# JohannesBuchner/massivedatans

Hardware: AMD Instinct MI355X
Metric: likelihood evals/sec across N datasets per constrained draw (higher is better)
Workload: dtype f64

## Files before the change

### massivedatans_amd/csrc/mdns_internal.h

```cpp
#pragma once
#include <hip/hip_runtime.h>
#include <cstddef>
#include <cstdint>
#include <cstring>
#include <utility>
#include "mdns.h"

namespace mdns {

void set_error(const char *fmt, ...);
bool hip_ok(hipError_t e, const char *what, const char *file, int line);
#define MDNS_HIP(call) ::mdns::hip_ok((call), #call, __FILE__, __LINE__)
bool launched(const char *name);

enum class Wait { ok, timeout, failed, empty };
Wait wait_seq(const volatile unsigned long long *at, unsigned long long want, hipError_t *err = nullptr);
bool wait_ok(Wait w, hipError_t err, const char *who);

constexpr size_t grown_bytes(size_t need, size_t elem) { return ((need + need / 2) * elem + 4095) / 4096 * 4096; }
static_assert(grown_bytes(0, 8) == 0, "nothing asked, nothing made");
static_assert(grown_bytes(1, 8) == 4096, "one element: one page");
static_assert(grown_bytes(341, 8) == 4096, "341 + 170 doubles = 4088 bytes: still one page");
static_assert(grown_bytes(342, 8) == 8192, "342 + 171 doubles = 4104 bytes: two pages");
constexpr size_t exact_bytes(size_t need, size_t elem) { return (need ? need : 1) * elem; }
// ... 132 lines not shown
	mdns_response *response = nullptr;
	mdns::DeviceBuffer<double> d_folded;
};

struct mdns_response {
	int nx = 0;
	int n_in = 0;
	long long nnz = 0;
	int attached = 0;
	mdns::DeviceBuffer<int> d_len;
	mdns::DeviceBuffer<long long> d_slice;
	mdns::DeviceBuffer<double> d_vals;
	mdns::DeviceBuffer<int> d_cols;
	mdns::DeviceBuffer<double> d_in, d_out;
};

struct mdns_table {
	int nx = 0;
	int d = 0;
	int nw = 0;
	int ndim = 0;
	int flags = 0;
	int n[MDNS_TABLE_MAX_AXES] = {};
	mdns::DeviceBuffer<double> d_x;
	mdns::DeviceBuffer<double> d_axes;
	mdns::DeviceBuffer<double> d_grid;
	mdns::DeviceBuffer<double> d_table;
	mdns::DeviceBuffer<double> d_ext;
	mdns::DeviceBuffer<double> d_delta;
	mdns::DeviceBuffer<double> d_params, d_out;
	mdns::DeviceBuffer<double> d_S, d_R;
};

namespace mdns {

bool launch_table_curves(mdns_table *t, const double *d_params, int B, double *d_out, int ldc);

bool launch_response_fold(const mdns_response *r, const double *d_curves, int ldc, int B, double *d_out, int ldo);
inline int curve_bins(const mdns_spectra *s) { return s->response ? s->response->n_in : s->nx; }
bool response_fold(mdns_spectra *s, const double **d_curves, int *ldc, int B);

inline int model_ld(int nx) { return nx <= 0 ? 512 : ((nx + 511) / 512) * 512; }

inline int cols_nx(int nx) { return ((nx + 7) / 8) * 8; }
bool ensure_model(mdns_spectra *s, size_t doubles);
bool ensure_selection(mdns_spectra *s, size_t doubles);
int gauss_loglike_cols_dev(mdns_spectra *s, const double *d_params, int B, double noise_level,
                           const int *d_row_ids, int M, double *d_Lout);
bool launch_gauss_model(const double *d_x, int nx, const double *d_params, int B,
                        double *d_model, int ldm);
int gauss_cols_tile(int M, int B);
bool launch_gauss_model_t(const double *d_x, int nx, const double *d_params, int B, int bt,
                          double *d_model_t, int *d_zero = nullptr, int nzero = 0);
struct JointArrays {
	double *live;
	double *shelfL;
	int *shelfn;
	double *higher;
	int nlive, cap, ndata;
};
struct JointHeader { int accepted; int status; long long pad; };
struct JointTrail {
	int *stamp_of;
	unsigned long long *word;
	double *L;
	int stamp;
};
struct JointMailbox { unsigned long long seq; int accepted; int status; unsigned long long bits[1];  };
bool chunk_fits(const mdns_spectra *s, int M, int B);
bool launch_chunk_accept(const mdns_spectra *s, const double *d_params_mapped, int B, double scale,
                         const int *d_rows_in, int *d_rows_dev, int M, const double *d_higher,
                         int *d_flags, int stamp, const JointTrail &trail, void *d_header);
bool launch_chunk_commit(const int *d_thr_rows, int M, int B, const int *d_flags, int stamp, const JointTrail &trail,
                         const JointArrays &st, void *d_header, unsigned long long *d_fillbits, void *box_dev,
                         unsigned long long seq);
bool launch_gauss_cols_accept(const mdns_spectra *s, const double *d_yT, const double *d_model_t, int bt, int B,
                              double scale, const int *d_rows, const int *d_thr_rows, int M,
                              const double *d_higher, int *d_flags, const JointTrail &trail);
int gauss_filter_pays(const mdns_spectra *s, int M, int B);
int gauss_filter_tile(int M, int B);
bool launch_gauss_model_tsq(const double *d_x, int nx, const double *d_params, int B, int bt, double *d_model_t, double *d_msq,
                            int *d_zero, int nzero, double *d_model_g = nullptr);
bool launch_gauss_cols_filter(const mdns_spectra *s, const double *d_yT, const double *d_model_t, int bt, int B,
                              double scale, const int *d_rows, const int *d_thr_rows, int M,
                              const double *d_higher, int *d_flags, const double *d_msq, const JointTrail &trail, int *d_lowest);
bool launch_row_sumsq(const double *d_y, int ld, int nx, int ndata, double *d_out);
#ifdef __HIPCC__
__host__ __device__
#endif
inline size_t tiled16_at(size_t r, int c, int ncp) { return (((r >> 4) * (size_t) ncp + (size_t) (c >> 1)) << 5) + ((r & 15) << 1) + (size_t) (c & 1); }
inline int tiled16_nx(int nx) { return (nx + 15) & ~15; }
bool launch_tile_rows16(const double *d_y, int ld, int M, int nx, const int *d_rows, double *d_out);
bool launch_gauss_mfma_filter(const mdns_spectra *s, const double *d_yT, const double *d_model_t, int B, double scale,
                              const int *d_thr_rows, int M, const double *d_higher, int *d_flags,
                              const double *d_msq, const JointTrail &trail, int *d_lowest, int *d_scratch, void *d_header,
                              const double *d_yG = nullptr, const double *d_model_g = nullptr);
int gauss_mfma_form();
bool launch_joint_commit_trail(const int *d_thr_rows, int M, int B, const int *d_flags, const JointTrail &trail,
                               const JointArrays &st, void *d_header, unsigned long long *d_fillbits, int flag_value = 1,
                               void *box_dev = nullptr, unsigned long long seq = 0, int *d_ticket = nullptr);
bool launch_gauss_cols_commit(const mdns_spectra *s, const double *d_yT, const double *d_model_t, int mstride, int B,
                              double scale, const int *d_rows, const int *d_thr_rows, int M, const int *d_flags,
                              const JointArrays &st, void *d_header, unsigned long long *d_fillbits, double *d_Lrow);
bool launch_gauss_cols(const mdns_spectra *s, const double *d_yT, const double *d_model_t, int bt, int B,
                       double scale, const int *d_rows, int M, double *d_out);
inline int muse_nparams(const mdns_spectra *s) { return s->nlines ? s->nlines + 2 : 5; }
bool launch_muse_model(const mdns_spectra *s, const double *d_params, int B, double *d_model, int ldm);
bool launch_gauss_rows(const mdns_spectra *s, const double *d_model, int ldm, int B,
                       double scale, const int *d_rows, int M, double *d_out);
struct MuseBandFused;
bool launch_muse_rows(const mdns_spectra *s, const double *d_model, int ldm, int B,
                      const int *d_rows, int M, double *d_out, int B_shape = 0, const MuseBandFused *band = nullptr);
// ... 65 lines not shown
	int nkept, B;
	int counts[kChainMost];
	double params[kChainMost][3];
	double u[kChainMost * kChainDim];
};
bool launch_box_count(const RegionView &rv, const ChainSpec &spec, ChainBox *box_dev, double *d_props, int *d_counts,
                      const CountMail *mail);
bool launch_chain_accept(const mdns_spectra *s, const ChainSpec &spec, const double *d_props, const int *d_counts,
                         ChainBox *box_dev, double scale, const int *d_rows_in, int *d_rows_dev, int M,
                         const double *d_higher, int *d_flags, int stamp, const JointTrail &trail, void *d_header);

struct ProfileScope {
	int slot;
	explicit ProfileScope(int which);
	~ProfileScope();
};
void note_kernel(int which, const char *fmt, ...);

#ifdef __HIPCC__
__device__ __forceinline__ void handover_release()
{
	__builtin_amdgcn_fence(__ATOMIC_RELEASE, "workgroup");
	asm volatile("s_waitcnt vmcnt(0)" ::: "memory");
}
__device__ __forceinline__ void handover_acquire() { __builtin_amdgcn_fence(__ATOMIC_ACQUIRE, "workgroup"); }
template <class T, class V> __device__ __forceinline__ void mail_store(T *at, V v) { __hip_atomic_store(at, (T) v, __ATOMIC_RELAXED, __HIP_MEMORY_SCOPE_SYSTEM); }
__device__ __forceinline__ void mail_raise(unsigned long long *seq_at, unsigned long long seq) { handover_release(); mail_store(seq_at, seq); }

template <int CTRL, int ROW_MASK>
__device__ __forceinline__ double dpp_move(double v)
{
	const int lo = __builtin_amdgcn_update_dpp(0, __double2loint(v), CTRL, ROW_MASK, 0xf, true);
	const int hi = __builtin_amdgcn_update_dpp(0, __double2hiint(v), CTRL, ROW_MASK, 0xf, true);
	return __hiloint2double(hi, lo);
}

__device__ __forceinline__ double wave_sum(double v)
{
	v += dpp_move<0xb1, 0xf>(v);
	v += dpp_move<0x4e, 0xf>(v);
	v += dpp_move<0x114, 0xf>(v);
	v += dpp_move<0x118, 0xf>(v);
	v += dpp_move<0x142, 0xa>(v);
	v += dpp_move<0x143, 0xc>(v);
	const int lo = __builtin_amdgcn_readlane(__double2loint(v), 63);
	const int hi = __builtin_amdgcn_readlane(__double2hiint(v), 63);
	return __hiloint2double(hi, lo);
}

template <int U>
__device__ __forceinline__ bool shelf_append(const JointArrays &st, int d, double L, double thr)
{
	const int n = st.shelfn[d];
	if (n >= st.cap) return false;
	int at_most = 0;
	double next = INFINITY;
	int p = 0;
	for (; p + U <= st.nlive; p += U) {
		double v[U];
#pragma unroll
		for (int u = 0; u < U; u++) v[u] = st.live[(size_t) (p + u) * st.ndata + d];
#pragma unroll
		for (int u = 0; u < U; u++) { if (v[u] <= thr) at_most++; else next = fmin(next, v[u]); }
	}
	for (; p < st.nlive; p++) {
		const double v = st.live[(size_t) p * st.ndata + d];
		if (v <= thr) at_most++; else next = fmin(next, v);
	}
	for (int e = 0; e < n; e++) {
		const double v = st.shelfL[(size_t) e * st.ndata + d];
		if (v <= thr) at_most++; else next = fmin(next, v);
	}
	st.shelfL[(size_t) n * st.ndata + d] = L;
	st.shelfn[d] = n + 1;
	st.higher[d] = at_most >= n + 2 ? thr : fmin(L, next);
	return true;
}

template <int BLOCK, class Flagged>
__device__ __forceinline__ int first_flagged(int *s_first, const int *__restrict__ flags, int B, Flagged flagged)
{
	if (threadIdx.x == 0) *s_first = 0x7fffffff;
	__syncthreads();
	for (int b = threadIdx.x; b < B; b += BLOCK)
		if (flagged(flags[b])) { atomicMin(s_first, b); break; }
	__syncthreads();
	return *s_first;
}

__device__ __forceinline__ unsigned long long trail_vote(const JointTrail &trail, int *__restrict__ flags, int cand, int B,
                                                         int ntiles, int tile, int lane, double L, double thr)
{
	const unsigned long long word = __ballot(L > thr);
	if (word != 0ull && cand < B) {
		const size_t at = (size_t) cand * ntiles + tile;
		if (trail.stamp_of) trail.L[at * 64 + lane] = L;
		if (lane == 0) {
			flags[cand] = 1;
			if (trail.stamp_of) { trail.word[at] = word; trail.stamp_of[at] = trail.stamp; }
		}
	}
	return word;
}
#endif


#ifdef __HIPCC__
static constexpr int kBandCap = 4096;
struct BandBox {
	unsigned long long seq;
	int npairs, pad;
	int status[MDNS_JOINT_MAX_BATCH];
	int pair_b[kBandCap], pair_k[kBandCap];
	double pair_L[kBandCap], pair_thr[kBandCap];
};
struct BandScratch {
	int counter, ticket;
	int clear[MDNS_JOINT_MAX_BATCH], maybe[MDNS_JOINT_MAX_BATCH];
	int pair_b[kBandCap], pair_k[kBandCap];
	double pair_L[kBandCap], pair_thr[kBandCap];
};

__device__ __forceinline__ void band_publish(BandScratch *__restrict__ sc, int B, BandBox *__restrict__ box, unsigned long long seq)
{
	const int n = __hip_atomic_load(&sc->counter, __ATOMIC_RELAXED, __HIP_MEMORY_SCOPE_AGENT);
// ... 44 lines not shown
```

### massivedatans_amd/csrc/mdns_joint.hip

```cpp
#include "mdns_internal.h"

#include <cmath>
#include <cstring>
#include <vector>

namespace mdns {

static constexpr int kBlock = 256;
static constexpr int kFlagInts = MDNS_JOINT_MAX_BATCH;
static constexpr int kZeroInts = kFlagInts + (int) (sizeof(JointHeader) / sizeof(int));

static constexpr int kSlices = 16, kHeld = 8;

template <typename T, typename F> __device__ __forceinline__ T over_slices(T v, F f)
{
	v = f(v, __shfl_xor(v, 4));
	v = f(v, __shfl_xor(v, 8));
	v = f(v, __shfl_xor(v, 16));
	v = f(v, __shfl_xor(v, 32));
	return v;
}

__global__ __launch_bounds__(kBlock) void k_joint_prepare(JointArrays st, const int *__restrict__ running, int nrun,
                                                          double *__restrict__ Lmin, int *__restrict__ argmin_run,
                                                          int *__restrict__ argmin, unsigned long long *__restrict__ keep,
                                                          int keep_words)
{
	const int lane = threadIdx.x & 63;
	const int q = lane & 3, sl = lane >> 2;
	const int r = (blockIdx.x * (kBlock / 64) + (threadIdx.x >> 6)) * 4 + q;
	const bool real = r < nrun;
	const int d = running[real ? r : nrun - 1];
	const size_t nd = (size_t) st.ndata;
	double lv[kHeld];
#pragma unroll
	for (int u = 0; u < kHeld; u++) {
		const int p = sl + kSlices * u;
		lv[u] = st.live[(size_t) (p < st.nlive ? p : 0) * nd + d];
	}
	const int n0 = st.shelfn[d];
	double sv[kHeld];
#pragma unroll
	for (int u = 0; u < kHeld; u++) {
		const int e = sl + kSlices * u;
		sv[u] = st.shelfL[(size_t) (e < n0 ? e : 0) * nd + d];
	}
	double m = INFINITY;
	int am = 0x7fffffff;
#pragma unroll
	for (int u = 0; u < kHeld; u++) if (sl + kSlices * u >= n0) sv[u] = __builtin_nan("");
#pragma unroll
	for (int u = 0; u < kHeld; u++) {
		const int p = sl + kSlices * u;
		if (p >= st.nlive) lv[u] = __builtin_nan("");
		if (lv[u] < m) { m = lv[u]; am = p; }
	}
	for (int p = sl + kSlices * kHeld; p < st.nlive; p += kSlices) { const double v = st.live[(size_t) p * nd + d]; if (v < m) { m = v; am = p; } }
	{
		const double mm = over_slices(m, [](double x, double y) { return y < x ? y : x; });
		am = over_slices(m == mm ? am : 0x7fffffff, [](int x, int y) { return y < x ? y : x; });
		m = mm;
		if (am == 0x7fffffff) am = 0;
	}
	const unsigned long long mine = 0x1111111111111111ull << q;
	const unsigned long long before = mine & ((1ull << lane) - 1ull);
	int w = 0;
	int w_held = -1;
	unsigned long long word = 0;
	for (int e0 = 0; e0 < keep_words * 64; e0 += kSlices) {
		const int e = e0 + sl;
		const int u = e0 / kSlices;
		if (u == kHeld) w_held = w;
		double v;
		if (u < kHeld) {
			v = sv[0];
#pragma unroll
			for (int k = 1; k < kHeld; k++) if (u == k) v = sv[k];
		} else v = st.shelfL[(size_t) (e < n0 ? e : 0) * nd + d];
		const bool kept = real && e < n0 && v > m;
		const unsigned long long votes = __ballot(kept) & mine;
		const int at = w + __popcll(votes & before);
		if (kept && at != e) st.shelfL[(size_t) at * nd + d] = v;
		if (kept) word |= 1ull << (e & 63);
		w += __popcll(votes);
		if (u < kHeld) {
#pragma unroll
			for (int k = 0; k < kHeld; k++) if (u == k && !kept) sv[k] = __builtin_nan("");
		}
		if (((e0 + kSlices) & 63) == 0) {
			const unsigned long long all = over_slices(word, [](unsigned long long x, unsigned long long y) { return x | y; });
			if (real && sl == 0) keep[(size_t) r * keep_words + (e0 >> 6)] = all;
			word = 0;
		}
	}
	if (real && sl == 0) st.shelfn[d] = w;
	if (w_held < 0) w_held = w;
	if (n0 > kSlices * kHeld) __threadfence();
	double thr = m;
	bool done = !real || w == 0;
	const int target = w + 1;
	const bool far = n0 > kSlices * kHeld || st.nlive > kSlices * kHeld;
	double lo = __builtin_nan(""), hi = __builtin_nan("");
	while (__any(!done)) {
		int inside = 0;
		double proposal = 0.0;
		auto in_range = [&](double v) { return v == v && !(v <= lo) && !(v >= hi); };
#pragma unroll
		for (int u = 0; u < kHeld; u++) inside += in_range(lv[u]);
#pragma unroll
		for (int u = 0; u < kHeld; u++) inside += in_range(sv[u]);
		if (far) {
			for (int p = sl + kSlices * kHeld; p < st.nlive; p += kSlices) inside += in_range(st.live[(size_t) p * nd + d]);
			for (int e = w_held + sl; e < w; e += kSlices) inside += in_range(st.shelfL[(size_t) e * nd + d]);
		}
		{
			int countdown = inside / 2;
			auto pick = [&](double v) { if (in_range(v) && countdown-- == 0) proposal = v; };
#pragma unroll
			for (int u = 0; u < kHeld; u++) pick(lv[u]);
#pragma unroll
			for (int u = 0; u < kHeld; u++) pick(sv[u]);
			if (far) {
				for (int p = sl + kSlices * kHeld; p < st.nlive; p += kSlices) pick(st.live[(size_t) p * nd + d]);
				for (int e = w_held + sl; e < w; e += kSlices) pick(st.shelfL[(size_t) e * nd + d]);
			}
		}
		const int most = over_slices(inside, [](int x, int y) { return y > x ? y : x; });
		const int from = over_slices(inside == most ? sl : kSlices, [](int x, int y) { return y < x ? y : x; });
		const double pivot = __shfl(proposal, 4 * from + q);
		if (!done && most == 0) {
			thr = hi == hi ? hi : INFINITY;
			done = true;
		}
		int count = 0;
#pragma unroll
		for (int u = 0; u < kHeld; u++) count += lv[u] <= pivot;
#pragma unroll
		for (int u = 0; u < kHeld; u++) count += sv[u] <= pivot;
		if (far) {
			for (int p = sl + kSlices * kHeld; p < st.nlive; p += kSlices) count += st.live[(size_t) p * nd + d] <= pivot;
			for (int e = w_held + sl; e < w; e += kSlices) count += st.shelfL[(size_t) e * nd + d] <= pivot;
		}
		const int total = over_slices(count, [](int x, int y) { return x + y; });
		if (!done) { if (total >= target) hi = pivot; else lo = pivot; }
	}
	if (!real || sl != 0) return;
	st.higher[d] = thr;
	Lmin[r] = m;
	argmin_run[r] = am;
	argmin[d] = am;
}

__global__ __launch_bounds__(kBlock) void k_joint_advance(JointArrays st, const int *__restrict__ running, int nrun,
                                                          const int *__restrict__ argmin, int *__restrict__ status)
{
	const int r = blockIdx.x * kBlock + threadIdx.x;
	if (r >= nrun) return;
	const int d = running[r];
	const size_t nd = (size_t) st.ndata;
	const int n = st.shelfn[d];
	if (n <= 0) { atomicOr(status, 1); return; }
	st.live[argmin[d] * nd + d] = st.shelfL[d];
	for (int e = 1; e < n; e++) st.shelfL[(e - 1) * nd + d] = st.shelfL[e * nd + d];
	st.shelfn[d] = n - 1;
}

__global__ __launch_bounds__(kBlock) void k_joint_undo_advance(JointArrays st, const int *__restrict__ running, int nrun,
                                                               const int *__restrict__ argmin, const double *__restrict__ Lmin)
{
	const int r = blockIdx.x * kBlock + threadIdx.x;
	if (r >= nrun) return;
	const int d = running[r];
	st.live[(size_t) argmin[d] * st.ndata + d] = Lmin[r];
	st.shelfn[d] = 0;
}

__global__ __launch_bounds__(kBlock) void k_joint_publish(const JointHeader *__restrict__ header,
                                                          const unsigned long long *__restrict__ fillbits, int nwords,
                                                          JointMailbox *__restrict__ box, unsigned long long seq)
{
	const int accepted = header->accepted;
	if (accepted >= 0)
		for (int w = threadIdx.x; w < nwords; w += kBlock) mail_store(&box->bits[w], fillbits[w]);
	handover_release();
	__syncthreads();
	if (threadIdx.x != 0) return;
	mail_store(&box->accepted, accepted);
	mail_store(&box->status, header->status);
	mail_raise(&box->seq, seq);
}

__global__ __launch_bounds__(kBlock) void k_joint_accept_dense(double *__restrict__ L, const double *__restrict__ jitter, int B, int M,
                                                               const int *__restrict__ thr_rows, const double *__restrict__ higher,
                                                               int *__restrict__ flags, int flag, JointHeader *__restrict__ header)
{
	if (blockIdx.x == 0 && blockIdx.y == 0 && threadIdx.x == 0) header->status = 0;
	const int k = blockIdx.x * kBlock + threadIdx.x, b = blockIdx.y;
	if (k >= M) return;
	const size_t at = (size_t) b * M + k;
// ... 46 lines not shown
	__syncthreads();
	if (!s_last) return;
	handover_acquire();
	band_publish(sc, B, box, seq);
}

__global__ __launch_bounds__(kBlock) void k_joint_band_publish(BandScratch *__restrict__ sc, int B, BandBox *__restrict__ box, unsigned long long seq)
{
	band_publish(sc, B, box, seq);
}

__global__ __launch_bounds__(kBlock) void k_joint_commit_band(
    const double *__restrict__ L, const double *__restrict__ jrow, const int *__restrict__ thr_rows, int M, int bstar, int ntiles,
    JointArrays st, JointHeader *__restrict__ header, unsigned long long *__restrict__ fillbits)
{
	if (blockIdx.x == 0 && threadIdx.x == 0) header->accepted = bstar;
	const int lane = threadIdx.x & 63;
	const int tile = blockIdx.x * (kBlock / 64) + (threadIdx.x >> 6);
	if (tile >= ntiles) return;
	const int k = tile * 64 + lane;
	bool beats = false;
	if (k < M) {
		const int d = thr_rows ? thr_rows[k] : k;
		const double v = L[(size_t) bstar * M + k] + jrow[k];
		const double thr = st.higher[d];
		beats = v > thr;
		if (beats && !shelf_append<20>(st, d, v, thr)) atomicOr(&header->status, 1);
	}
	const unsigned long long word = __ballot(beats);
	if (lane == 0) fillbits[tile] = word;
}

__global__ void k_joint_add(double *__restrict__ p, const double *__restrict__ q, size_t n)
{
	for (size_t e = (size_t) blockIdx.x * blockDim.x + threadIdx.x; e < n; e += (size_t) gridDim.x * blockDim.x) p[e] = p[e] + q[e];
}

__global__ void k_joint_fill(double *__restrict__ p, size_t n, double value)
{
	for (size_t e = (size_t) blockIdx.x * blockDim.x + threadIdx.x; e < n; e += (size_t) gridDim.x * blockDim.x) p[e] = value;
}

}

using namespace mdns;

struct ChunkScore { int path, B, flag; };

struct mdns_joint {
	mdns_spectra *s = nullptr;
	int nlive = 0, cap = 0, ndata = 0;
	DeviceBuffer<double> live, shelfL, higher;
	DeviceBuffer<int> shelfn;
	JointArrays st = {};
	DeviceBuffer<int> d_running;  int nrun = 0;
	DeviceBuffer<double> d_Lmin;
	DeviceBuffer<int> d_argmin_run;
	DeviceBuffer<int> d_argmin;
	DeviceBuffer<unsigned long long> d_keep;
	DeviceBuffer<int> d_status;
	DeviceBuffer<int> d_flags;
	char *d_result = nullptr;
	PinnedBuffer box{hipHostMallocMapped | hipHostMallocCoherent};
	JointMailbox *h_box = nullptr, *h_box_dev = nullptr;
	unsigned long long box_seq = 0;
	bool box_pending = false;
	DeviceBuffer<int> d_trail_stamp;  DeviceBuffer<unsigned long long> d_trail_word;  DeviceBuffer<double> d_trail_L;
	int trail_stamp = 0;
	bool trail_valid = false;
	DeviceBuffer<char> d_params;
	double *params() const { return (double *) d_params.get(); }
	int *d_rows = nullptr;
	PinnedBuffer h_pin;
	const double *last_yT = nullptr;
	const int *last_gather = nullptr;
	int last_bt = 0, last_B = 0;
	double last_scale = 0;
	bool prepared = false;
	bool staged_rows = false;
	bool staged_valid = false;
	int scored_M = -1;
	int staged_M = 0;
	size_t staged_in_bytes = 0;
	double noise_level = 0;
	CurveStat stat = kCurveNoise;
	int nparams = 3;
	bool counted = false;
	DeviceBuffer<double> d_msq;
	DeviceBuffer<int> d_filter_scratch;
	DeviceBuffer<double> d_dense;
	DeviceBuffer<double> d_jitter;
	DeviceBuffer<double> d_curves;
	DeviceBuffer<double> d_tparams;
	DeviceBuffer<int> d_sel_rows;
	bool sel_rows = false;
	int sel_M = 0;
	bool sel_open = false;
	bool sel_on_device = false;
	int chunk_seq = 1;
	PinnedBuffer in_block{hipHostMallocMapped};
	char *h_in = nullptr, *h_in_dev = nullptr;
	int shelf_bound = 0;
	PinnedBuffer chain_box{hipHostMallocMapped};
	ChainBox *h_chain = nullptr, *h_chain_dev = nullptr;
	DeviceBuffer<double> d_chain_props;
	DeviceBuffer<int> d_chain_counts, d_chain_ticket;
	DeviceBuffer<int> d_commit_ticket;
	PinnedBuffer band_box{hipHostMallocMapped};
	BandBox *h_band = nullptr, *h_band_dev = nullptr;
	DeviceBuffer<BandScratch> d_band;
	DeviceBuffer<double> d_bound;
	unsigned long long band_seq = 0;
	int band_B = 0;
	bool band_pending = false;
	bool band_exact = true;
	DeviceBuffer<int> d_votes;
	ChunkScore half = {0, 0, 0};
	unsigned long long chain_seq = 0;
	int chain_state = 0;
	int chain_n = 0;
};

static size_t result_bytes(int M) { return sizeof(JointHeader) + (size_t) ((M + 63) / 64) * 8 + (size_t) M * 8; }
extern "C" size_t mdns_joint_result_bytes(int M) { return result_bytes(M > 0 ? M : 0); }
static int keep_words_of(int cap) { return (cap + 63) / 64; }

static bool joint_sync(Context *c) { return MDNS_HIP(hipStreamSynchronize(c->stream)); }

extern "C" void mdns_joint_destroy(mdns_joint *j)
{
	if (!j) return;
	Context *c = ctx();
	if (c) (void) hipStreamSynchronize(c->stream);
	if (j->s && j->counted) j->s->njoint--;
	delete j;
}

extern "C" mdns_joint *mdns_joint_create(mdns_spectra *s, int nlive, int shelf_cap)
{
	Context *c = ctx();
	if (!c) return nullptr;
	if (!s || nlive <= 0 || s->ndata <= 0) { set_error("mdns_joint_create: bad arguments (nlive=%d)", nlive); return nullptr; }
	if (!s->d_x.get() || (!s->d_yT.get() && !s->d_w.get())) { set_error("mdns_joint_create: the spectra need a wavelength grid"); return nullptr; }
	if (shelf_cap < 4) shelf_cap = 4;
	mdns_joint *j = new mdns_joint();
	j->s = s; j->nlive = nlive; j->cap = shelf_cap; j->ndata = s->ndata;
	j->stat = curve_stat(s);
	j->nparams = j->stat == kCurveMarginal ? muse_nparams(s) : 3;
	const size_t nd = (size_t) s->ndata;
	const size_t res = (size_t) kFlagInts * sizeof(int) + result_bytes(s->ndata);
	static_assert(sizeof(JointHeader) % sizeof(int) == 0, "d_flags is counted in ints");
	bool ok =
	    j->live.make((size_t) nlive * nd) && j->shelfL.make((size_t) shelf_cap * nd) && j->shelfn.make(nd) && j->higher.make(nd) &&
	    j->d_running.make(nd) && j->d_Lmin.make(nd) && j->d_argmin_run.make(nd) && j->d_argmin.make(nd) && j->d_status.make(1) &&
	    j->d_flags.make(res / sizeof(int)) &&
	    j->d_params.make((size_t) MDNS_JOINT_MAX_BATCH * kJointParamsMost * sizeof(double) + nd * sizeof(int) + 16) &&
	    j->box.make(sizeof(JointMailbox) + ((nd + 63) / 64) * 8);
	if (ok) {
		j->h_box = (JointMailbox *) j->box.get(); j->h_box_dev = (JointMailbox *) j->box.dev();
		j->d_result = (char *) (j->d_flags.get() + kFlagInts);
		j->st = {j->live.get(), j->shelfL.get(), j->shelfn.get(), j->higher.get(), nlive, shelf_cap, s->ndata};
		std::vector<int> all(nd);
		for (size_t i = 0; i < nd; i++) all[i] = (int) i;
		ok = MDNS_HIP(hipMemsetAsync(j->st.shelfn, 0, nd * sizeof(int), c->stream)) &&
		     MDNS_HIP(hipMemsetAsync(j->d_status.get(), 0, sizeof(int), c->stream)) &&
		     MDNS_HIP(hipMemsetAsync(j->d_flags.get(), 0, res, c->stream)) &&
		     MDNS_HIP(hipMemsetAsync(j->d_argmin.get(), 0, nd * sizeof(int), c->stream)) &&
		     MDNS_HIP(hipMemcpyAsync(j->d_running.get(), all.data(), nd * sizeof(int), hipMemcpyHostToDevice, c->stream));
		if (ok) {
			hipLaunchKernelGGL(k_joint_fill, dim3(256), dim3(kBlock), 0, c->stream, j->st.higher, nd, (double) NAN);
			ok = MDNS_HIP(hipGetLastError()) && joint_sync(c);
		}
		j->nrun = s->ndata;
	}
	if (!ok) { mdns_joint_destroy(j); return nullptr; }
	s->njoint++;
	j->counted = true;
	return j;
}

extern "C" int mdns_joint_shelf_cap(const mdns_joint *j) { return j ? j->cap : -1; }
extern "C" int mdns_joint_keep_words(const mdns_joint *j) { return j ? keep_words_of(j->cap) : -1; }

extern "C" int mdns_joint_reserve(mdns_joint *j, int shelf_cap)
{
	Context *c = ctx();
	if (!c || !j) return 1;
	if (shelf_cap <= j->cap) return 0;
	int cap = j->cap;
	while (cap < shelf_cap) cap *= 2;
	const size_t nd = (size_t) j->ndata;
	DeviceBuffer<double> bigger;
	if (!bigger.make((size_t) cap * nd)) return 1;
	if (!MDNS_HIP(hipMemcpyAsync(bigger.get(), j->st.shelfL, (size_t) j->cap * nd * sizeof(double), hipMemcpyDeviceToDevice, c->stream)) ||
	    !joint_sync(c)) return 1;
	j->shelfL = std::move(bigger);
	j->st.shelfL = j->shelfL.get();
	j->cap = j->st.cap = cap;
	return 0;
}

static int joint_reset(mdns_joint *j)
{
	Context *c = ctx();
	j->prepared = false;
	j->shelf_bound = 0;
	return MDNS_HIP(hipMemsetAsync(j->st.shelfn, 0, (size_t) j->ndata * sizeof(int), c->stream)) &&
	       MDNS_HIP(hipMemsetAsync(j->d_status.get(), 0, sizeof(int), c->stream)) ? 0 : 1;
}

enum : unsigned { kTakesLine = 1, kTakesTemplate = 2, kNamesNull = 4, kBandIdle = 8 };
static bool wrong_stat(const mdns_joint *j, unsigned takes, const char *who, const char *other)
{
	if (j->stat == kCurveNoise || j->stat == kCurveMarginal) {
		if (takes & (j->stat == kCurveNoise ? kTakesLine : kTakesTemplate)) return false;
		set_error("%s: %s", who, other);
		return true;
	}
	set_error("%s: %s spectra take curve chunks only (mdns_joint_init_curves, mdns_backend_draw_curves)", who,
	          j->stat == kCurveChi2 ? "fixed-scale" : "counts");
	return true;
}

static bool stage_h2d(mdns_joint *j, Context *c, void *dst, const void *src, size_t bytes, const void *src2 = nullptr, size_t bytes2 = 0,
                      size_t room = 0)
{
	const size_t all = bytes + bytes2;
	if (!j->h_pin.fit(room > all ? room : all)) return false;
	if (all == 0) return true;
	char *pin = j->h_pin.get();
	if (bytes) memcpy(pin, src, bytes);
	if (bytes2) memcpy(pin + bytes, src2, bytes2);
	return MDNS_HIP(hipMemcpyAsync(dst, pin, all, hipMemcpyHostToDevice, c->stream));
}

static const double *chunk_noise(mdns_joint *j, Context *c, const double *jitter, size_t n)
{
	if (!jitter || !j->d_jitter.fit(n) ||
	    !MDNS_HIP(hipMemcpyAsync(j->d_jitter.get(), jitter, n * sizeof(double), hipMemcpyHostToDevice, c->stream))) return nullptr;
	return j->d_jitter.get();
}

static bool add_noise_to_live(mdns_joint *j, Context *c, const double *jitter)
{
	const size_t n = (size_t) j->nlive * j->ndata;
	const double *d_noise = chunk_noise(j, c, jitter, n);
	if (!d_noise) return !jitter;
	hipLaunchKernelGGL(k_joint_add, dim3(1024), dim3(kBlock), 0, c->stream, j->st.live, d_noise, n);
	return MDNS_HIP(hipGetLastError());
}

static int init_finish(mdns_joint *j, Context *c, const double *jitter)
{
	return add_noise_to_live(j, c, jitter) && joint_reset(j) == 0 && joint_sync(c) ? 0 : 1;
}

extern "C" int mdns_joint_init_gauss(mdns_joint *j, const double *params, double noise_level)
{
	Context *c = ctx();
// ... 42 lines not shown
	if (j->stat == kCurveNoise) j->noise_level = noise_level;
	if (!j->d_curves.fit((size_t) j->nlive * nx)) return 1;
	if (!MDNS_HIP(hipMemcpyAsync(j->d_curves.get(), curves, (size_t) j->nlive * nx * sizeof(double), hipMemcpyHostToDevice, c->stream))) return 1;
	return init_from_curves(j, c, jitter);
}

static bool table_fits(const mdns_joint *j, const mdns_table *table, const char *who)
{
	if (!table) { set_error("%s: null table handle", who); return false; }
	if (j->s->response && table->nx != j->s->response->n_in) {
		set_error("%s: the table model makes curves of %d bins, the spectra's response takes %d", who, table->nx, j->s->response->n_in);
		return false;
	}
	if (!j->s->response && table->nx != j->s->nx) {
		set_error("%s: the table model makes curves of %d channels, the spectra have %d", who, table->nx, j->s->nx);
		return false;
	}
	return true;
}

static bool table_curves(mdns_joint *j, Context *c, mdns_table *table, const double *params, int B)
{
	const size_t np = (size_t) B * table->ndim;
	return j->d_tparams.fit(np) && j->d_curves.fit((size_t) B * table->nx) &&
	       MDNS_HIP(hipMemcpyAsync(j->d_tparams.get(), params, np * sizeof(double), hipMemcpyHostToDevice, c->stream)) &&
	       launch_table_curves(table, j->d_tparams.get(), B, j->d_curves.get(), table->nx);
}

extern "C" int mdns_joint_init_table(mdns_joint *j, mdns_table *table, const double *params, double noise_level, const double *jitter)
{
	Context *c = ctx();
	if (!c || !j || !params) return 1;
	if (j->s->nx < 1) { set_error("mdns_joint_init_table: spectra without channels"); return 1; }
	if (!table_fits(j, table, "mdns_joint_init_table")) return 1;
	if (j->stat == kCurveNoise) j->noise_level = noise_level;
	if (!table_curves(j, c, table, params, j->nlive)) return 1;
	return init_from_curves(j, c, jitter);
}

extern "C" int mdns_joint_restore_live_dev(mdns_joint *j, const double *d_liveL)
{
	Context *c = ctx();
	if (!c || !j || !d_liveL) return 1;
	if (!MDNS_HIP(hipMemcpyAsync(j->st.live, d_liveL, (size_t) j->nlive * j->ndata * sizeof(double), hipMemcpyDeviceToDevice, c->stream))) return 1;
	return joint_reset(j);
}

extern "C" int mdns_joint_undo_advance_dev(mdns_joint *j)
{
	Context *c = ctx();
	if (!c || !j) return 1;
	if (!j->prepared) { set_error("mdns_joint_undo_advance_dev: nothing to take back"); return 1; }
	if (j->nrun == 0) return 0;
	hipLaunchKernelGGL(k_joint_undo_advance, dim3((j->nrun + kBlock - 1) / kBlock), dim3(kBlock), 0, c->stream,
	                   j->st, j->d_running.get(), j->nrun, j->d_argmin.get(), j->d_Lmin.get());
	return MDNS_HIP(hipGetLastError()) ? 0 : 1;
}

extern "C" const double *mdns_joint_live_dev(mdns_joint *j) { return j ? j->st.live : nullptr; }

extern "C" int mdns_joint_set_live(mdns_joint *j, const double *liveL)
{
	Context *c = ctx();
	if (!c || !j || !liveL) return 1;
	if (!MDNS_HIP(hipMemcpyAsync(j->st.live, liveL, (size_t) j->nlive * j->ndata * sizeof(double), hipMemcpyHostToDevice, c->stream))) return 1;
	if (joint_reset(j) != 0) return 1;
	return joint_sync(c) ? 0 : 1;
}

extern "C" int mdns_joint_get_live(mdns_joint *j, double *liveL)
{
	Context *c = ctx();
	if (!c || !j || !liveL) return 1;
	if (!MDNS_HIP(hipMemcpyAsync(liveL, j->st.live, (size_t) j->nlive * j->ndata * sizeof(double), hipMemcpyDeviceToHost, c->stream))) return 1;
	return joint_sync(c) ? 0 : 1;
}

extern "C" int mdns_joint_get_thresholds(mdns_joint *j, double *higher, int *shelf_n)
{
	Context *c = ctx();
	if (!c || !j) return 1;
	if (higher && !MDNS_HIP(hipMemcpyAsync(higher, j->st.higher, (size_t) j->ndata * sizeof(double), hipMemcpyDeviceToHost, c->stream))) return 1;
	if (shelf_n && !MDNS_HIP(hipMemcpyAsync(shelf_n, j->st.shelfn, (size_t) j->ndata * sizeof(int), hipMemcpyDeviceToHost, c->stream))) return 1;
	return joint_sync(c) ? 0 : 1;
}

extern "C" int mdns_joint_set_running(mdns_joint *j, const int *rows, int nrun)
{
	Context *c = ctx();
	if (!c || !j) return 1;
	if (nrun < 0 || nrun > j->ndata || (nrun > 0 && !rows)) { set_error("mdns_joint_set_running: nrun=%d", nrun); return 1; }
	for (int i = 0; i < nrun; i++)
		if (rows[i] < 0 || rows[i] >= j->ndata || (i > 0 && rows[i] <= rows[i - 1])) {
			set_error("mdns_joint_set_running: rows must be ascending indices below %d", j->ndata);
			return 1;
		}
	if (nrun > 0 && (!MDNS_HIP(hipMemcpyAsync(j->d_running.get(), rows, (size_t) nrun * sizeof(int), hipMemcpyHostToDevice, c->stream)) ||
	                 !joint_sync(c))) return 1;
	j->nrun = nrun;
	return 0;
}

extern "C" int mdns_joint_prepare_dev(mdns_joint *j)
{
	Context *c = ctx();
	if (!c || !j) return 1;
	const int kw = keep_words_of(j->cap);
	if (!j->d_keep.fit((size_t) j->ndata * kw)) return 1;
	j->prepared = true;
	if (j->nrun == 0) return 0;
	hipLaunchKernelGGL(k_joint_prepare, dim3((j->nrun + 15) / 16), dim3(kBlock), 0, c->stream,
	                   j->st, j->d_running.get(), j->nrun, j->d_Lmin.get(), j->d_argmin_run.get(), j->d_argmin.get(), j->d_keep.get(), kw);
	return MDNS_HIP(hipGetLastError()) ? 0 : 1;
}

extern "C" int mdns_joint_prepare(mdns_joint *j, double *Lmin, int *argmin, unsigned long long *keep)
{
	Context *c = ctx();
	if (mdns_joint_prepare_dev(j) != 0) return 1;
	const int kw = keep_words_of(j->cap);
	const size_t n = (size_t) j->nrun;
	if (n == 0) return 0;
	const size_t o1 = n * 8, o2 = o1 + ((n * 4 + 7) & ~(size_t) 7);
	if (!j->h_pin.fit(o2 + n * kw * 8)) return 1;
	char *pin = j->h_pin.get();
	if (!MDNS_HIP(hipMemcpyAsync(pin, j->d_Lmin.get(), n * 8, hipMemcpyDeviceToHost, c->stream)) ||
	    !MDNS_HIP(hipMemcpyAsync(pin + o1, j->d_argmin_run.get(), n * 4, hipMemcpyDeviceToHost, c->stream)) ||
	    !MDNS_HIP(hipMemcpyAsync(pin + o2, j->d_keep.get(), n * kw * 8, hipMemcpyDeviceToHost, c->stream)) ||
	    !joint_sync(c)) return 1;
	if (Lmin) memcpy(Lmin, pin, n * 8);
	if (argmin) memcpy(argmin, pin + o1, n * 4);
	if (keep) memcpy(keep, pin + o2, n * kw * 8);
	int longest = 0;
	const unsigned long long *kwords = (const unsigned long long *) (pin + o2);
	for (size_t r = 0; r < n; r++) {
		int kept = 0;
		for (int w = 0; w < kw; w++) kept += __builtin_popcountll(kwords[r * kw + w]);
		if (kept > longest) longest = kept;
	}
	j->shelf_bound = longest;
	return 0;
}

extern "C" int mdns_joint_advance_dev(mdns_joint *j)
{
	Context *c = ctx();
	if (!c || !j) return 1;
	if (!j->prepared) { set_error("mdns_joint_advance: no prepare since the state was set"); return 1; }
	if (j->nrun == 0) return 0;
	hipLaunchKernelGGL(k_joint_advance, dim3((j->nrun + kBlock - 1) / kBlock), dim3(kBlock), 0, c->stream,
	                   j->st, j->d_running.get(), j->nrun, j->d_argmin.get(), j->d_status.get());
	return MDNS_HIP(hipGetLastError()) ? 0 : 1;
}

extern "C" int mdns_joint_advance(mdns_joint *j)
{
	Context *c = ctx();
	if (mdns_joint_advance_dev(j) != 0) return 1;
	int status = 0;
	if (!MDNS_HIP(hipMemcpyAsync(&status, j->d_status.get(), sizeof(int), hipMemcpyDeviceToHost, c->stream)) || !joint_sync(c)) return 1;
	if (status) { set_error("mdns_joint_advance: a running data set had an empty shelf"); return 1; }
	if (j->shelf_bound > 0) j->shelf_bound--;
	return 0;
}

static bool joint_trail(mdns_joint *j, int B, int M, JointTrail *out)
{
	Context *c = ctx();
	const size_t need = (size_t) B * ((M + 63) / 64);
	const size_t had = j->d_trail_stamp.cap();
	if (!j->d_trail_stamp.fit_zeroed(need)) { j->trail_valid = false; return false; }
	if (j->d_trail_stamp.cap() != had) j->trail_stamp = 0;
	if (!j->d_trail_word.fit(need) || !j->d_trail_L.fit(need * 64)) { j->trail_valid = false; return false; }
	if (j->trail_stamp == 0x7fffffff) {
		if (!MDNS_HIP(hipMemsetAsync(j->d_trail_stamp.get(), 0, j->d_trail_stamp.cap() * sizeof(int), c->stream))) return false;
		j->trail_stamp = 0;
	}
	out->stamp_of = j->d_trail_stamp.get(); out->word = j->d_trail_word.get(); out->L = j->d_trail_L.get();
	out->stamp = ++j->trail_stamp;
	return true;
}

static void status_error(const char *who, int status, int cap)
{
	if (status & 2) set_error("%s: more ambiguous candidates than the exact pass lists (guarded filter)", who);
	else set_error("%s: a shelf overflowed its capacity %d (mdns_joint_reserve)", who, cap);
}

static bool check_draw(const mdns_joint *j, int B, int M, const char *who)
{
	if (!j) { set_error("%s: null handle", who); return false; }
	if (B < 0 || B > MDNS_JOINT_MAX_BATCH || M < 0 || M > j->ndata) {
		set_error("%s: bad sizes B=%d (<= %d) M=%d (ndata=%d)", who, B, MDNS_JOINT_MAX_BATCH, M, j->ndata);
		return false;
	}
	return true;
}

extern "C" int mdns_joint_score_dev(mdns_joint *j, const double *d_params, int B, double noise_level,
                                    const int *d_row_ids, int M)
{
	Context *c = ctx();
// ... 796 lines not shown
```

### massivedatans_amd/csrc/mdns_like.hip

```cpp
#include "mdns_internal.h"
#include <climits>
#include <cstdlib>

namespace mdns {

static constexpr int kBlock = 256;


__device__ __forceinline__ double swap_add32(double a, double b)
{
	const auto lo = __builtin_amdgcn_permlane32_swap((unsigned) __double2loint(a), (unsigned) __double2loint(b), false, false);
	const auto hi = __builtin_amdgcn_permlane32_swap((unsigned) __double2hiint(a), (unsigned) __double2hiint(b), false, false);
	return __hiloint2double((int) hi[0], (int) lo[0]) + __hiloint2double((int) hi[1], (int) lo[1]);
}
__device__ __forceinline__ double swap_add16(double a, double b)
{
	const auto lo = __builtin_amdgcn_permlane16_swap((unsigned) __double2loint(a), (unsigned) __double2loint(b), false, false);
	const auto hi = __builtin_amdgcn_permlane16_swap((unsigned) __double2hiint(a), (unsigned) __double2hiint(b), false, false);
	return __hiloint2double((int) hi[0], (int) lo[0]) + __hiloint2double((int) hi[1], (int) lo[1]);
}
__device__ __forceinline__ double row_sum(double v)
{
	v += dpp_move<0xb1, 0xf>(v);
	v += dpp_move<0x4e, 0xf>(v);
// ... 521 lines not shown
	const double yy = ysq[d];
	const double unit = fabs(scale) * (double) (nx + 8) * 0x1p-52;
	unsigned hits = 0, maybes = 0;
#pragma unroll
	for (int b = 0; b < BT; b++) {
		const int cand = bt * BT + b;
		const double mm = msq[cand];
		const double Lf = scale * ((mm - 2.0 * acc[0][b]) + yy);
		const double E4 = 4.0 * unit * ((mm + 2.0 * fabs(acc[0][b])) + yy);
		const bool valid = cand < B;
		if (__ballot(valid && Lf > thr + E4) != 0ull) hits |= 1u << b;
		else if (__ballot(valid && Lf >= thr - E4) != 0ull) maybes |= 1u << b;
	}
	unsigned todo = hits | maybes;
#pragma unroll 1
	while (todo) {
		const int b = __builtin_ctz(todo);
		todo &= todo - 1;
		const int cand = bt * BT + b;
		const int seen = B - __hip_atomic_load(lowest, __ATOMIC_RELAXED, __HIP_MEMORY_SCOPE_AGENT);
		if ((hits >> b & 1u) && cand > seen) { if (lane == 0) flags[cand] = 1; continue; }
		int k1[1];
		double a1[1][1];
		cols_accumulate<1, 1, true>(YT, nxp, mp + b, BT, rows, M, tile, lane, k1, a1);
		const unsigned long long word = trail_vote(trail, flags, cand, B, ntiles, tile, lane, a1[0][0] * scale, thr);
		if (word != 0ull && lane == 0) atomicMax(lowest, B - cand);
	}
}

__global__ void k_row_sumsq(const double *__restrict__ Y, int ld, int nx, int ndata, double *__restrict__ out)
{
	const int i = blockIdx.x * blockDim.x + threadIdx.x;
	if (i >= ndata) return;
	const double *yr = Y + (size_t) i * ld;
	double acc = 0.0;
	for (int j = 0; j < nx; j++) acc = fma(yr[j], yr[j], acc);
	out[i] = acc;
}

__global__ __launch_bounds__(kBlock) void k_joint_commit_trail(
    const int *__restrict__ thr_rows, int M, int B, int ntiles, const int *__restrict__ flags, int flag_value, JointTrail trail,
    JointArrays st, JointHeader *__restrict__ header, unsigned long long *__restrict__ fillbits,
    JointMailbox *__restrict__ box, unsigned long long seq, int *__restrict__ ticket)
{
	__shared__ int s_first;
	__shared__ int s_last;
	const int bstar = first_flagged<kBlock>(&s_first, flags, B, [=](int f) { return f == flag_value; });
	if (blockIdx.x == 0 && threadIdx.x == 0) header->accepted = bstar < B ? bstar : -1;
	const int lane = threadIdx.x & 63;
	const int tile = blockIdx.x * (kBlock / 64) + (threadIdx.x >> 6);
	const bool mine = bstar < B && tile < ntiles;
	if (!mine && !box) return;
	const size_t at = mine ? (size_t) bstar * ntiles + tile : 0;
	const unsigned long long word = mine && trail.stamp_of[at] == trail.stamp ? trail.word[at] : 0ull;
	const int k = tile * 64 + lane;
	if (mine && k < M && (word >> lane & 1ull)) {
		const int d = thr_rows ? thr_rows[k] : k;
		if (!shelf_append<25>(st, d, trail.L[at * 64 + lane], st.higher[d])) atomicOr(&header->status, 1);
	}
	if (!box) { if (lane == 0) fillbits[tile] = word; return; }
	if (mine && lane == 0) __hip_atomic_store(&fillbits[tile], word, __ATOMIC_RELAXED, __HIP_MEMORY_SCOPE_AGENT);
	handover_release();
	__syncthreads();
	if (threadIdx.x == 0) s_last = atomicAdd(ticket, 1) == (int) gridDim.x - 1 ? 1 : 0;
	__syncthreads();
	if (!s_last) return;
	handover_acquire();
	if (bstar < B)
		for (int w = threadIdx.x; w < ntiles; w += kBlock)
			mail_store(&box->bits[w], __hip_atomic_load(&fillbits[w], __ATOMIC_RELAXED, __HIP_MEMORY_SCOPE_AGENT));
	handover_release();
	__syncthreads();
	if (threadIdx.x != 0) return;
	*ticket = 0;
	mail_store(&box->accepted, bstar < B ? bstar : -1);
	mail_store(&box->status, __hip_atomic_load(&header->status, __ATOMIC_RELAXED, __HIP_MEMORY_SCOPE_AGENT));
	mail_raise(&box->seq, seq);
}

__global__ __launch_bounds__(kBlock) void k_gauss_cols_commit(
    const double *__restrict__ YT, int nxp, const double *__restrict__ model_t, int mstride, int B,
    double scale, const int *__restrict__ rows, const int *__restrict__ thr_rows, int M,
    int ntiles, int nq_xcd, int cu_slots, const int *__restrict__ flags, JointArrays st,
    JointHeader *__restrict__ header, unsigned long long *__restrict__ fillbits, double *__restrict__ Lrow)
{
	extern __shared__ __attribute__((aligned(16))) double tpl[];
	const int bstar = first_flagged<kBlock>(reinterpret_cast<int *>(tpl + nxp), flags, B, [](int f) { return f != 0; });
	if (blockIdx.x == 0 && threadIdx.x == 0) header->accepted = bstar < B ? bstar : -1;
	if (bstar >= B) return;
	const int lane = threadIdx.x & 63;
	int tile, bt_unused;
	if (!cols_item(ntiles, INT_MAX, nq_xcd, 1, cu_slots, tile, bt_unused)) return;
	stage_templates(tpl, model_t + (size_t) (bstar / mstride) * nxp * mstride + bstar % mstride, nxp, mstride);
	if (tile >= ntiles) return;
	int k[1];
	double acc[1][1];
	cols_accumulate_deep<1, 4>(YT, nxp, tpl, rows, M, tile, lane, k[0], acc[0]);
	const bool live = k[0] < M;
	const double L = acc[0][0] * scale;
	bool beats = false;
	if (live) {
		const int d = thr_rows ? thr_rows[k[0]] : k[0];
		Lrow[k[0]] = L;
		const double thr = st.higher[d];
		beats = L > thr;
		if (beats && !shelf_append<8>(st, d, L, thr)) atomicOr(&header->status, 1);
	}
	const unsigned long long word = __ballot(beats);
	if (lane == 0) fillbits[tile] = word;
}

// ... 586 lines not shown
```

Baseline: 29.09 billion.

## Cache per-dataset live-point count and next-higher value across prepare and commit

The prepare kernel now computes, for each running dataset, how many live points lie at or below the threshold and the smallest value above it, and stores these in a per-dataset record tagged with an epoch. shelf_append reuses that record when the epoch and threshold match, skipping the full scan over live points, and scans only the shelf. The commit kernel also issues its trail, L and row-id loads before the branch. Host calls bump the epoch on each state change to invalidate stale records, at the cost of extra work in prepare and an extra per-dataset array.

```diff
diff --git a/massivedatans_amd/csrc/mdns_internal.h b/massivedatans_amd/csrc/mdns_internal.h
--- a/massivedatans_amd/csrc/mdns_internal.h
+++ b/massivedatans_amd/csrc/mdns_internal.h
@@ -208,12 +208,20 @@
 int gauss_cols_tile(int M, int B);
 bool launch_gauss_model_t(const double *d_x, int nx, const double *d_params, int B, int bt,
                           double *d_model_t, int *d_zero = nullptr, int nzero = 0);
+struct alignas(32) JointRecord {
+	double key;
+	double next;
+	unsigned long long epoch;
+	int cnt, pad;
+};
 struct JointArrays {
 	double *live;
 	double *shelfL;
 	int *shelfn;
 	double *higher;
 	int nlive, cap, ndata;
+	JointRecord *rec;
+	unsigned long long epoch;
 };
 struct JointHeader { int accepted; int status; long long pad; };
 struct JointTrail {
@@ -385,25 +393,31 @@
 __device__ __forceinline__ bool shelf_append(const JointArrays &st, int d, double L, double thr)
 {
 	const int n = st.shelfn[d];
-	if (n >= st.cap) return false;
+	const JointRecord rec = st.rec[d];
 	int at_most = 0;
 	double next = INFINITY;
-	int p = 0;
-	for (; p + U <= st.nlive; p += U) {
-		double v[U];
+	if (rec.epoch == st.epoch && rec.key == thr) {
+		at_most = rec.cnt;
+		next = rec.next;
+	} else {
+		int p = 0;
+		for (; p + U <= st.nlive; p += U) {
+			double v[U];
 #pragma unroll
-		for (int u = 0; u < U; u++) v[u] = st.live[(size_t) (p + u) * st.ndata + d];
+			for (int u = 0; u < U; u++) v[u] = st.live[(size_t) (p + u) * st.ndata + d];
 #pragma unroll
-		for (int u = 0; u < U; u++) { if (v[u] <= thr) at_most++; else next = fmin(next, v[u]); }
-	}
-	for (; p < st.nlive; p++) {
-		const double v = st.live[(size_t) p * st.ndata + d];
-		if (v <= thr) at_most++; else next = fmin(next, v);
+			for (int u = 0; u < U; u++) { if (v[u] <= thr) at_most++; else next = fmin(next, v[u]); }
+		}
+		for (; p < st.nlive; p++) {
+			const double v = st.live[(size_t) p * st.ndata + d];
+			if (v <= thr) at_most++; else next = fmin(next, v);
+		}
 	}
 	for (int e = 0; e < n; e++) {
 		const double v = st.shelfL[(size_t) e * st.ndata + d];
 		if (v <= thr) at_most++; else next = fmin(next, v);
 	}
+	if (n >= st.cap) return false;
 	st.shelfL[(size_t) n * st.ndata + d] = L;
 	st.shelfn[d] = n + 1;
 	st.higher[d] = at_most >= n + 2 ? thr : fmin(L, next);
diff --git a/massivedatans_amd/csrc/mdns_joint.hip b/massivedatans_amd/csrc/mdns_joint.hip
--- a/massivedatans_amd/csrc/mdns_joint.hip
+++ b/massivedatans_amd/csrc/mdns_joint.hip
@@ -43,7 +43,7 @@
 #pragma unroll
 	for (int u = 0; u < kHeld; u++) {
 		const int e = sl + kSlices * u;
-		sv[u] = st.shelfL[(size_t) (e < n0 ? e : 0) * nd + d];
+		sv[u] = st.shelfL[(size_t) (e < st.cap ? e : 0) * nd + d];
 	}
 	double m = INFINITY;
 	int am = 0x7fffffff;
@@ -144,7 +144,16 @@
 		const int total = over_slices(count, [](int x, int y) { return x + y; });
 		if (!done) { if (total >= target) hi = pivot; else lo = pivot; }
 	}
+	int cnt = 0;
+	double next = INFINITY;
+	auto note = [&](double v) { if (v <= thr) cnt++; else next = fmin(next, v); };
+#pragma unroll
+	for (int u = 0; u < kHeld; u++) note(lv[u]);
+	for (int p = sl + kSlices * kHeld; p < st.nlive; p += kSlices) note(st.live[(size_t) p * nd + d]);
+	cnt = over_slices(cnt, [](int x, int y) { return x + y; });
+	next = over_slices(next, [](double x, double y) { return fmin(x, y); });
 	if (!real || sl != 0) return;
+	st.rec[d] = JointRecord{thr, next, st.epoch, cnt, 0};
 	st.higher[d] = thr;
 	Lmin[r] = m;
 	argmin_run[r] = am;
@@ -297,6 +306,7 @@
 	int nlive = 0, cap = 0, ndata = 0;
 	DeviceBuffer<double> live, shelfL, higher;
 	DeviceBuffer<int> shelfn;
+	DeviceBuffer<JointRecord> rec;
 	JointArrays st = {};
 	DeviceBuffer<int> d_running;  int nrun = 0;
 	DeviceBuffer<double> d_Lmin;
@@ -366,6 +376,8 @@
 	int chain_n = 0;
 };
 
+static void joint_new_epoch(mdns_joint *j) { j->st.epoch++; }
+
 static size_t result_bytes(int M) { return sizeof(JointHeader) + (size_t) ((M + 63) / 64) * 8 + (size_t) M * 8; }
 extern "C" size_t mdns_joint_result_bytes(int M) { return result_bytes(M > 0 ? M : 0); }
 static int keep_words_of(int cap) { return (cap + 63) / 64; }
@@ -396,7 +408,7 @@
 	const size_t res = (size_t) kFlagInts * sizeof(int) + result_bytes(s->ndata);
 	static_assert(sizeof(JointHeader) % sizeof(int) == 0, "d_flags is counted in ints");
 	bool ok =
-	    j->live.make((size_t) nlive * nd) && j->shelfL.make((size_t) shelf_cap * nd) && j->shelfn.make(nd) && j->higher.make(nd) &&
+	    j->live.make((size_t) nlive * nd) && j->shelfL.make((size_t) shelf_cap * nd) && j->shelfn.make(nd) && j->higher.make(nd) && j->rec.make(nd) &&
 	    j->d_running.make(nd) && j->d_Lmin.make(nd) && j->d_argmin_run.make(nd) && j->d_argmin.make(nd) && j->d_status.make(1) &&
 	    j->d_flags.make(res / sizeof(int)) &&
 	    j->d_params.make((size_t) MDNS_JOINT_MAX_BATCH * kJointParamsMost * sizeof(double) + nd * sizeof(int) + 16) &&
@@ -404,10 +416,11 @@
 	if (ok) {
 		j->h_box = (JointMailbox *) j->box.get(); j->h_box_dev = (JointMailbox *) j->box.dev();
 		j->d_result = (char *) (j->d_flags.get() + kFlagInts);
-		j->st = {j->live.get(), j->shelfL.get(), j->shelfn.get(), j->higher.get(), nlive, shelf_cap, s->ndata};
+		j->st = {j->live.get(), j->shelfL.get(), j->shelfn.get(), j->higher.get(), nlive, shelf_cap, s->ndata, j->rec.get(), 1};
 		std::vector<int> all(nd);
 		for (size_t i = 0; i < nd; i++) all[i] = (int) i;
 		ok = MDNS_HIP(hipMemsetAsync(j->st.shelfn, 0, nd * sizeof(int), c->stream)) &&
+		     MDNS_HIP(hipMemsetAsync(j->st.rec, 0, nd * sizeof(JointRecord), c->stream)) &&
 		     MDNS_HIP(hipMemsetAsync(j->d_status.get(), 0, sizeof(int), c->stream)) &&
 		     MDNS_HIP(hipMemsetAsync(j->d_flags.get(), 0, res, c->stream)) &&
 		     MDNS_HIP(hipMemsetAsync(j->d_argmin.get(), 0, nd * sizeof(int), c->stream)) &&
@@ -450,6 +463,7 @@
 	Context *c = ctx();
 	j->prepared = false;
 	j->shelf_bound = 0;
+	joint_new_epoch(j);
 	return MDNS_HIP(hipMemsetAsync(j->st.shelfn, 0, (size_t) j->ndata * sizeof(int), c->stream)) &&
 	       MDNS_HIP(hipMemsetAsync(j->d_status.get(), 0, sizeof(int), c->stream)) ? 0 : 1;
 }
@@ -598,6 +612,7 @@
 	if (!c || !j) return 1;
 	if (!j->prepared) { set_error("mdns_joint_undo_advance_dev: nothing to take back"); return 1; }
 	if (j->nrun == 0) return 0;
+	joint_new_epoch(j);
 	hipLaunchKernelGGL(k_joint_undo_advance, dim3((j->nrun + kBlock - 1) / kBlock), dim3(kBlock), 0, c->stream,
 	                   j->st, j->d_running.get(), j->nrun, j->d_argmin.get(), j->d_Lmin.get());
 	return MDNS_HIP(hipGetLastError()) ? 0 : 1;
@@ -655,6 +670,7 @@
 	if (!j->d_keep.fit((size_t) j->ndata * kw)) return 1;
 	j->prepared = true;
 	if (j->nrun == 0) return 0;
+	joint_new_epoch(j);
 	hipLaunchKernelGGL(k_joint_prepare, dim3((j->nrun + 15) / 16), dim3(kBlock), 0, c->stream,
 	                   j->st, j->d_running.get(), j->nrun, j->d_Lmin.get(), j->d_argmin_run.get(), j->d_argmin.get(), j->d_keep.get(), kw);
 	return MDNS_HIP(hipGetLastError()) ? 0 : 1;
@@ -694,6 +710,7 @@
 	if (!c || !j) return 1;
 	if (!j->prepared) { set_error("mdns_joint_advance: no prepare since the state was set"); return 1; }
 	if (j->nrun == 0) return 0;
+	joint_new_epoch(j);
 	hipLaunchKernelGGL(k_joint_advance, dim3((j->nrun + kBlock - 1) / kBlock), dim3(kBlock), 0, c->stream,
 	                   j->st, j->d_running.get(), j->nrun, j->d_argmin.get(), j->d_status.get());
 	return MDNS_HIP(hipGetLastError()) ? 0 : 1;
diff --git a/massivedatans_amd/csrc/mdns_like.hip b/massivedatans_amd/csrc/mdns_like.hip
--- a/massivedatans_amd/csrc/mdns_like.hip
+++ b/massivedatans_amd/csrc/mdns_like.hip
@@ -597,11 +597,19 @@
 	const bool mine = bstar < B && tile < ntiles;
 	if (!mine && !box) return;
 	const size_t at = mine ? (size_t) bstar * ntiles + tile : 0;
-	const unsigned long long word = mine && trail.stamp_of[at] == trail.stamp ? trail.word[at] : 0ull;
 	const int k = tile * 64 + lane;
+	int stamp = 0, d = 0;
+	unsigned long long entry = 0ull;
+	double L = 0.0;
+	if (mine) {
+		stamp = trail.stamp_of[at];
+		entry = trail.word[at];
+		L = trail.L[at * 64 + lane];
+		if (k < M) d = thr_rows ? thr_rows[k] : k;
+	}
+	const unsigned long long word = mine && stamp == trail.stamp ? entry : 0ull;
 	if (mine && k < M && (word >> lane & 1ull)) {
-		const int d = thr_rows ? thr_rows[k] : k;
-		if (!shelf_append<25>(st, d, trail.L[at * 64 + lane], st.higher[d])) atomicOr(&header->status, 1);
+		if (!shelf_append<25>(st, d, L, st.higher[d])) atomicOr(&header->status, 1);
 	}
 	if (!box) { if (lane == 0) fillbits[tile] = word; return; }
 	if (mine && lane == 0) __hip_atomic_store(&fillbits[tile], word, __ATOMIC_RELAXED, __HIP_MEMORY_SCOPE_AGENT);
```

Result: faster. 31.11 billion (median of 6 runs) (+6.9%).
